# tesseract-robotics/trajopt

Hardware: NVIDIA H100
Metric: converged trajectories/sec (7-DOF x 30 wp, batch 1024) (higher is better)
Workload: dtype f64

## Files before the change

trajopt_b200/csrc/qp_cta_kernel.cuh:

```cuda
#pragma once
#include "device_types.cuh"
#include "joint_terms.cuh"

namespace tb200 {

#ifdef TB200_PROFILE
static __device__ unsigned long long g_prof[32];
#define PROF_T0() const long long prof_t0_ = clock64()
#define PROF_ADD(slot) do { if (q.tid == 0) atomicAdd(&g_prof[slot], (unsigned long long)(clock64() - prof_t0_)); } while (0)
#define PROF_COUNT(slot) do { if (q.tid == 0) atomicAdd(&g_prof[slot], 1ull); } while (0)
#else
#define PROF_T0()
#define PROF_ADD(slot)
#define PROF_COUNT(slot)
#endif
#if defined(TB200_PROFILE) && defined(TB200_PROFILE_CHECK)
#define PROF_CHK_T0() long long pc_ = clock64()
#define PROF_CHK(slot) do { const long long n_ = clock64(); if (q.tid == 0) atomicAdd(&g_prof[slot], (unsigned long long)(n_ - pc_)); pc_ = n_; } while (0)
#else
#define PROF_CHK_T0()
#define PROF_CHK(slot)
#endif

constexpr int kQpThreads = 256;
// ... 709 lines not shown
      if (mine && R.bu_store) w[R.bu_dst] = acc + o;
    }
    __syncthreads();
  }
  if (wbase < R.b0_warps) {
    const double acc = reg_bwd_task<NB>(mB0, (side ? w : v) + R.b0_y, w + R.b0_wl, side, R.b0_hasl, R.b0_hasr);
    const double o = __shfl_xor_sync(0xffffffffu, acc, 1);
    if (R.b0_store) w[R.b0_dst] = acc + o;
  }
  __syncthreads();
}

template <int NB>
__device__ __forceinline__ double p_row(const QpCtx& q, const int i, const double* Dz, const double* vin) {
  constexpr int HB = NB, W = HB + 1;
  const int N = q.N, nbo = q.n_band;
  const double* const Pb = q.Pband;
  const int* const offs = q.band_offs;
  double s = 0.0;
  for (int t0 = 0; t0 < nbo; t0 += 4) {
    double v[4];
#pragma unroll
    for (int u = 0; u < 4; ++u) {
      const int k = (t0 + u < nbo) ? offs[t0 + u] : -1;
      v[u] = (k >= 0 && k <= i) ? (Pb[i * W + k] * Dz[i - k]) * vin[i - k] : 0.0;
    }
    s += v[0]; s += v[1]; s += v[2]; s += v[3];
  }
  for (int t0 = 0; t0 < nbo; t0 += 4) {
    double v[4];
#pragma unroll
    for (int u = 0; u < 4; ++u) {
      const int k = (t0 + u < nbo) ? offs[t0 + u] : -1;
      v[u] = (k >= 1 && i + k < N) ? (Pb[(i + k) * W + k] * Dz[i + k]) * vin[i + k] : 0.0;
    }
    s += v[0]; s += v[1]; s += v[2]; s += v[3];
  }
  return s * (q.c * Dz[i]);
}
template <int NB>
__device__ __forceinline__ void p_matvec(const QpCtx& q, const double* in, double* out) {
  extern __shared__ double sm[];
  const int N = q.N, Np = q.Np;
  const double* const Dz = sm + (q.Dz - q.smbase);
  const double* const vin = sm + (in - q.smbase);
  double* const vout = sm + (out - q.smbase);
  for (int i = q.tid; i < Np; i += kQpThreads) vout[i] = (i < N) ? p_row<NB>(q, i, Dz, vin) : 0.0;
  __syncthreads();
}

__device__ __forceinline__ void info_row_terms(const double* F, const double ax, double (&m)[14]) {
  const double einv = 1.0 / F[R_E];
  m[0] = fmax(m[0], fabs(einv * (ax - F[R_Z])));
  m[1] = fmax(m[1], fabs(einv * F[R_Z]));
  m[2] = fmax(m[2], fabs(einv * ax));
  m[7] = fmax(m[7], fabs(ax - F[R_Z]));
  m[8] = fmax(m[8], fabs(F[R_Z]));
  m[9] = fmax(m[9], fabs(ax));
#pragma unroll
  for (int k = 0; k < 2; ++k) {
    const double u = F[R_U0 + k], bb = F[R_B0 + k], qa = F[R_QA0 + k];
    const double xa = F[R_XA0 + k], za = F[R_ZA0 + k], ya = F[R_YA0 + k];
    const double iea = 1.0 / F[R_EA0 + k], ida = 1.0 / F[R_DA0 + k];
    const double axb = bb * xa;
    m[0] = fmax(m[0], fabs(iea * (axb - za)));
    m[1] = fmax(m[1], fabs(iea * za));
    m[2] = fmax(m[2], fabs(iea * axb));
    m[7] = fmax(m[7], fabs(axb - za));
    m[8] = fmax(m[8], fabs(za));
    m[9] = fmax(m[9], fabs(axb));
    const double aty = u * F[R_Y] + bb * ya;
    m[3] = fmax(m[3], fabs(ida * (qa + aty)));
    m[4] = fmax(m[4], fabs(ida * aty));
    m[5] = fmax(m[5], fabs(ida * qa));
    m[10] = fmax(m[10], fabs(qa + aty));
    m[11] = fmax(m[11], fabs(aty));
    m[12] = fmax(m[12], fabs(qa));
  }
}
__device__ __forceinline__ void info_var_terms(const double dz, const double beta, const double x, const double zb,
                                               const double aty, const double px, const double qv, double (&m)[14]) {
  const double ax = beta * x;
  const double einv = dz / beta, dinv = 1.0 / dz;
  m[0] = fmax(m[0], fabs(einv * (ax - zb)));
  m[1] = fmax(m[1], fabs(einv * zb));
  m[2] = fmax(m[2], fabs(einv * ax));
  m[7] = fmax(m[7], fabs(ax - zb));
  m[8] = fmax(m[8], fabs(zb));
  m[9] = fmax(m[9], fabs(ax));
  const double d = qv + px + aty;
  m[3] = fmax(m[3], fabs(dinv * d));
  m[4] = fmax(m[4], fabs(dinv * aty));
  m[5] = fmax(m[5], fabs(dinv * qv));
  m[6] = fmax(m[6], fabs(dinv * px));
  m[10] = fmax(m[10], fabs(d));
  m[11] = fmax(m[11], fabs(aty));
  m[12] = fmax(m[12], fabs(qv));
  m[13] = fmax(m[13], fabs(px));
}
__device__ __forceinline__ double pinf_row_terms(const double* F, const int naux, double (&a)[3]) {
  double d = F[R_DY];
  d = (naux == AUX_HINGE) ? fmax(d, 0.0) : d;
  a[0] = fmax(a[0], fabs(F[R_E] * d));
  a[1] += F[R_UP] * fmax(d, 0.0) + F[R_LO] * fmin(d, 0.0);
#pragma unroll
  for (int k = 0; k < 2; ++k) {
    const double da = fmin(F[R_DYA0 + k], 0.0);
    a[0] = fmax(a[0], fabs(F[R_EA0 + k] * da));
    a[2] = fmax(a[2], fabs((F[R_U0 + k] * d + F[R_B0 + k] * da) / F[R_DA0 + k]));
  }
  return d;
}
__device__ __forceinline__ void pinf_var_terms(const double ratio, const double ub, const double lb, const double d,
                                               double (&a)[3]) {
  a[0] = fmax(a[0], fabs(ratio * d));
  a[1] += ub * fmax(d, 0.0) + lb * fmin(d, 0.0);
}
__device__ __forceinline__ void dinf_row_terms(const double* F, double (&a)[2]) {
#pragma unroll
  for (int k = 0; k < 2; ++k) {
    a[0] = fmax(a[0], fabs(F[R_DA0 + k] * F[R_DXA0 + k]));
    a[1] += F[R_QA0 + k] * F[R_DXA0 + k];
  }
}
__device__ __forceinline__ unsigned long long guess_mix(unsigned long long v) {
  v += 0x9e3779b97f4a7c15ull;
  v = (v ^ (v >> 30)) * 0xbf58476d1ce4e5b9ull;
  v = (v ^ (v >> 27)) * 0x94d049bb133111ebull;
  return v ^ (v >> 31);
}
__device__ __forceinline__ unsigned long long guess_row_hash(const double* F, const int* I, const int r, const int nrows,
                                                             const int N) {
  unsigned long long h = 0ull;
  const unsigned long long mc = static_cast<unsigned long long>(nrows);
  if (F[R_Z] - F[R_LO] < -F[R_Y]) h += guess_mix(2ull * r);
  else if (F[R_UP] - F[R_Z] < F[R_Y]) h += guess_mix(2ull * r + 1ull);
  for (int k = 0; k < I[RI_AUX]; ++k) {
    const unsigned long long idx = mc + N + I[RI_PAD] + k;
    if (F[R_ZA0 + k] - 0.0 < -F[R_YA0 + k]) h += guess_mix(2ull * idx);
    else if (kOsqpInf * F[R_EA0 + k] - F[R_ZA0 + k] < F[R_YA0 + k]) h += guess_mix(2ull * idx + 1ull);
  }
  return h;
}
__device__ __forceinline__ unsigned long long guess_var_hash(const double zb, const double yb, const double lb,
                                                             const double ub, const int i, const int nrows) {
  const unsigned long long idx = static_cast<unsigned long long>(nrows) + i;
  if (zb - lb < -yb) return guess_mix(2ull * idx);
  if (ub - zb < yb) return guess_mix(2ull * idx + 1ull);
  return 0ull;
}
enum ChkQ { CHK_PA0 = 14, CHK_PA1, CHK_PA2, CHK_DA0, CHK_DA1, kChkHash };
constexpr unsigned kChkSumMask = (1u << CHK_PA1) | (1u << CHK_DA1);

__device__ inline void rows_prepare_weights(const QpCtx& q, const SysW& w) {
  for (int r = q.tid; r < q.nrows; r += kQpThreads) {
    double* F = q.F(r);
    const int naux = q.I(r)[RI_AUX];
    const double Wr = w.polish ? fabs(F[R_PW]) : ((F[R_RHO] != 0.0) ? q.rho_eq : q.rho);
    const double wa0 = w.polish ? fabs(F[R_PWA0]) : w.rho_aux;
    const double wa1 = w.polish ? fabs(F[R_PWA1]) : w.rho_aux;
    const double g0 = (naux >= 1) ? w.sig + wa0 * F[R_B0] * F[R_B0] : 1.0;
    const double g1 = (naux == 2) ? w.sig + wa1 * F[R_B1] * F[R_B1] : 1.0;
    const double den = g0 * g1 + Wr * (F[R_U0] * F[R_U0] * g1 + F[R_U1] * F[R_U1] * g0);
    F[R_WRR] = Wr;
    F[R_G0] = g0;
    F[R_G1] = g1;
    F[R_DEN] = den;
    F[R_IDEN] = 1.0 / den;
    F[R_IWRR] = (Wr != 0.0) ? 1.0 / Wr : 0.0;
    F[R_WR] = Wr * g0 * g1 / den;
  }
  __syncthreads();
}
__device__ __forceinline__ double xbound_weight(const QpCtx& q, const SysW& w, int j) {
  const double adm = (q.ubs[j] - q.lbs[j] < kRhoTol) ? q.rho_eq : q.rho;
  return w.polish ? fabs(q.zb[j]) : adm;
}

__device__ __forceinline__ double pivot_rcp(const double x) {
  double r;
  asm("rcp.approx.ftz.f64 %0, %1;" : "=d"(r) : "d"(x));
  double e = fma(-x, r, 1.0);
  r = fma(r, e, r);
  e = fma(-x, r, 1.0);
  r = fma(r, e, r);
  e = fma(-x, r, 1.0);
  return fma(r, e, r);
}
template <int QN>
__device__ __forceinline__ bool gj_rows(double (&a)[QN], double diag, const bool active, const int mat, const int row,
                                        const int n, const int n_max, double* tmp, const int nmat) {
  constexpr int BS = QN + 2;
  double* const csv = tmp + 2 * nmat * BS + mat * QN;
  bool bad = false;
  double pv_mine = pivot_rcp(diag), my_cs = 1.0, rs = 1.0, inv_rs = 1.0;
#pragma unroll 1
  for (int k = 0; k < n_max; ++k) {
    double* buf = tmp + ((k & 1) * nmat + mat) * BS;
    const bool piv = active && row == k;
    if (piv) {
      bad |= !(diag > 0.0);
#pragma unroll
      for (int j = 0; j < QN; j += 2) *reinterpret_cast<double2*>(buf + j) = make_double2(a[j], a[j + 1]);
      buf[k] = 0.0;
      buf[QN] = pv_mine;
      my_cs = -pv_mine;
      csv[k] = my_cs;
      rs = pv_mine;
      inv_rs = diag;
      diag = pv_mine;
    }
    __syncthreads();
    if (active && k < n && !piv) {
      const double tr = buf[row];
      const bool ahead = row > k;
      const double f = ahead ? tr : -tr * my_cs;
      const double g = f * buf[QN];
      diag = ahead ? diag - g * f : diag + g * f;
      const double gs = g * inv_rs;
#pragma unroll
      for (int j = 0; j < QN; j += 2) {
        const double2 t = *reinterpret_cast<const double2*>(buf + j);
        a[j] -= gs * t.x;
        a[j + 1] -= gs * t.y;
      }
      if (ahead) pv_mine = pivot_rcp(diag);
    }
  }
  if (active) {
#pragma unroll
    for (int j = 0; j < QN; ++j) a[j] = (j == row) ? diag : ((j < n) ? a[j] * (rs * csv[j]) : 0.0);
  }
  return bad;
}

template <int NB>
__device__ inline bool pinv_factor(const QpCtx& q) {
  constexpr int QN = 3 * NB, blk = NB * NB;
  static_assert(QN % 2 == 0, "pivot rows move as double2");
  extern __shared__ double sm[];
  const int tid = q.tid, M = q.M, Np = q.Np;
  const int PR = q.pl.PR, nS = q.pl.nS, Ns = q.pl.Ns, ZS = q.pl.ZS, WS = q.pl.WS, SS = q.pl.SS;
  double* const fbase = sm + (q.SA - q.smbase);
  const double* const SA = fbase;
  const double* const SLM = sm + (q.SLM - q.smbase);
  double* const Z = fbase + q.pl.zo;
  double* const W = fbase + q.pl.wo;
  double* const S = fbase + q.pl.so;
  double* const tmp = q.tmp.ptr();
  const int nparts = (M + 3) / 4;
  bool bad = false;
#ifdef TB200_PROFILE
  long long pf_ = clock64();
#define PROF_PF(slot) do { const long long n_ = clock64(); if (tid == 0) atomicAdd(&g_prof[slot], (unsigned long long)(n_ - pf_)); pf_ = n_; } while (0)
#else
#define PROF_PF(slot)
#endif
  {
    const bool prow = tid < PR;
    const int p = prow ? tid / QN : 0, lr = prow ? tid % QN : 0;
    const int npb = (M - 4 * p) < 3 ? (M - 4 * p) : 3;
    const int kb = lr / NB, r = lr % NB, gb = 4 * p + kb;
    double a[QN];
#pragma unroll
    for (int j = 0; j < QN; ++j) {
      const int cb = j / NB, c = j % NB;
      double v = 0.0;
      if (prow && cb < npb) {
        if (cb == kb) v = SA[gb * blk + r * NB + c];
        else if (cb == kb - 1) v = SLM[gb * blk + r * NB + c];
        else if (cb == kb + 1) v = SLM[(gb + 1) * blk + c * NB + r];
      }
      a[j] = v;
    }
    PROF_PF(0);
    const double dg = prow ? SA[gb * blk + r * NB + r] : 1.0;
    bad |= gj_rows<QN>(a, dg, prow, p, lr, npb * NB, (M < 3 ? M : 3) * NB, tmp, nparts);
    PROF_PF(4);
    if (prow) {
#pragma unroll
      for (int j = 0; j < QN; ++j) q.pi_g[tid * QN + j] = a[j];
      const bool has_l = p > 0, has_r = 4 * p + 3 < M;
#pragma unroll 2
      for (int j = 0; j < NB; ++j) {
        double wl = 0.0, wr = 0.0;
        if (has_l) {
#pragma unroll
          for (int c = 0; c < NB; ++c) wl += a[c] * SLM[(4 * p) * blk + c * NB + j];
        }
        if (has_r) {
#pragma unroll
          for (int c = 0; c < NB; ++c) wr += a[2 * NB + c] * SLM[(4 * p + 3) * blk + j * NB + c];
        }
        W[tid * WS + j] = wl;
        W[tid * WS + NB + j] = wr;
      }
    }
  }
  __syncthreads();
  for (int e = tid; e < nS * nS; e += kQpThreads) {
    const int ra = e / nS, ca = e % nS, sa = ra / NB, i = ra % NB, sb = ca / NB, j = ca % NB;
    double v = 0.0;
    if (sa == sb || sb == sa + 1 || sb == sa - 1) {
      const bool use_l = sb <= sa, use_r = sb >= sa && 4 * sa + 4 < M;
      const double* cl = SLM + (4 * sa + 3) * blk + i * NB;
      const double* wl = W + (sa * QN + 2 * NB) * WS + (sb == sa ? NB : 0) + j;
      const double* cr = SLM + (4 * sa + 4) * blk + i;
      const double* wr = W + ((sa + 1) * QN) * WS + (sb == sa ? 0 : NB) + j;
      double s0 = 0.0, s1 = 0.0, s2 = 0.0, s3 = 0.0;
      if (use_l) {
#pragma unroll
        for (int rr = 0; rr < NB; rr += 2) {
          s0 += cl[rr] * wl[rr * WS];
          s1 += cl[rr + 1] * wl[(rr + 1) * WS];
        }
      }
      if (use_r) {
#pragma unroll
        for (int rr = 0; rr < NB; rr += 2) {
          s2 += cr[rr * NB] * wr[rr * WS];
          s3 += cr[(rr + 1) * NB] * wr[(rr + 1) * WS];
        }
      }
      v = ((sa == sb) ? SA[(4 * sa + 3) * blk + i * NB + j] : 0.0) - ((s0 + s1) + (s2 + s3));
    }
    S[ra * SS + ca] = v;
  }
  __syncthreads();
  PROF_PF(14);
  {
    const bool srow = tid < nS;
    double a[QN];
#pragma unroll
    for (int j = 0; j < QN; ++j) a[j] = (srow && j < nS) ? S[tid * SS + j] : 0.0;
    const double dg = srow ? S[tid * SS + tid] : 1.0;
    bad |= gj_rows<QN>(a, dg, srow, 0, tid, nS, nS, tmp, 1);
    if (srow) {
#pragma unroll
      for (int j = 0; j < QN; ++j)
        if (j < nS) S[tid * SS + j] = a[j];
    }
  }
  __syncthreads();
  PROF_PF(15);
  if (tid < Np) {
    const int col = tid, cb = col / NB, c = col % NB, p = cb / 4;
    if (cb % 4 == 3) {
      for (int sr = 0; sr < nS; ++sr) Z[sr * ZS + col] = S[sr * SS + p * NB + c];
    } else {
      const bool has_l = p > 0, has_r = 4 * p + 3 < M;
      const double* wrow = W + (p * QN + (cb % 4) * NB + c) * WS;
      double wv[2 * NB];
#pragma unroll
      for (int t = 0; t < 2 * NB; ++t) wv[t] = wrow[t];
      const double* sl = S + (has_l ? (p - 1) * NB : 0);
      const double* sr_ = S + (has_r ? p * NB : 0);
#pragma unroll 2
      for (int sr = 0; sr < nS; ++sr) {
        double s0 = 0.0, s1 = 0.0, s2 = 0.0, s3 = 0.0;
#pragma unroll
        for (int t = 0; t < NB; t += 2) {
          s0 += sl[sr * SS + t] * wv[t];
          s1 += sl[sr * SS + t + 1] * wv[t + 1];
          s2 += sr_[sr * SS + t] * wv[NB + t];
          s3 += sr_[sr * SS + t + 1] * wv[NB + t + 1];
        }
        Z[sr * ZS + col] = -((s0 + s1) + (s2 + s3));
      }
    }
  }
  (void)Ns;
  const bool ok = !__syncthreads_or(bad ? 1 : 0);
  PROF_PF(9);
  return ok;
}

template <int NB, bool PINV>
__device__ __noinline__ bool assemble_factor(const QpCtx& q, const SysW& w) {
  PROF_T0();
  rows_prepare_weights(q, w);
  constexpr int nb = NB, blk = NB * NB;
  const int N = q.N, HB = 2 * q.D, PW = HB + 1, CN = q.CN;
  for (int t = q.tid; t < q.M * blk; t += kQpThreads) {
    q.SA[t] = 0.0;
    q.SLM[t] = 0.0;
  }
  __syncthreads();
  for (int i = q.tid; i < q.Np; i += kQpThreads) {
    const int p = i / nb, r = i % nb;
    double* Arow = q.SA + static_cast<size_t>(p) * blk + r * nb;
    double* Lrow = q.SLM + static_cast<size_t>(p) * blk + r * nb;
    if (i >= N) {
      Arow[r] = 1.0;
      continue;
    }
    auto add = [&](int k, double val) {
      if (k <= r) Arow[r - k] += val;
      else Lrow[nb + r - k] += val;
    };
    for (int t = 0; t < q.n_band; ++t) {
      const int k = q.band_offs[t];
      if (k <= i) add(k, q.c * q.Dz[i] * q.Pband[i * PW + k] * q.Dz[i - k]);
    }
    add(0, w.sig + xbound_weight(q, w, i) * q.beta[i] * q.beta[i]);
    for (int e = q.colptr[i]; e < q.colptr[i + 1]; ++e) {
      const int ent = q.colent[e], rw = ent >> 5, k = ent & 31;
      const double* R = q.R(rw);
      const double wr = R[2 * CN + R_WR];
      if (wr == 0.0) continue;
      const int stride = q.I(rw)[RI_STRIDE];
      const double* as = R + CN;
      const double ai = wr * as[k];
      for (int k2 = 0; k2 <= k; ++k2) add((k - k2) * stride, ai * as[k2]);
    }
  }
  __syncthreads();
  for (int t = q.tid; t < q.M * blk; t += kQpThreads) {
    const int p = t / blk, i = (t % blk) / nb, j = t % nb;
    if (j > i) q.SA[static_cast<size_t>(p) * blk + i * nb + j] = q.SA[static_cast<size_t>(p) * blk + j * nb + i];
  }
  __syncthreads();
  PROF_ADD(10);
  bool ok;
  {
    PROF_T0();
    if constexpr (PINV) ok = pinv_factor<NB>(q);
    else ok = bcr_factor<NB>(q);
    PROF_ADD(11);
  }
  return ok;
}

struct QpPlan {
  bool use_reg, use_pinv, fuse, fast_polish;
};
__host__ __device__ inline QpPlan qp_plan(bool regok, int pinv, int rows_smem, int M, int nb, bool fast_passes) {
  QpPlan pl;
  pl.use_reg = regok && solve_roles_fit(M, nb);
  pl.use_pinv = regok && pinv && rows_smem;
  pl.fuse = pl.use_pinv && fast_passes;
  pl.fast_polish = pl.use_pinv && fast_passes && M * nb <= kQpThreads && solve_roles_fit(M, nb);
  return pl;
}
enum QpPath {
  QPP_BLOCK_PINV = 1 << 0,
  QPP_BLOCK_FAST = 1 << 1,
  QPP_BLOCK_GENERIC = 1 << 2,
  QPP_BLOCK_SOA = 1 << 3,
  QPP_FACTOR_GLOBAL = 1 << 4,
  QPP_BAND_GLOBAL = 1 << 5,
  QPP_ROWS_GLOBAL = 1 << 6,
  QPP_FUSED_CHECK = 1 << 7,
  QPP_POLISH_FAST = 1 << 8,
  QPP_POLISH_GENERIC = 1 << 9
};
__host__ __device__ inline int qp_plan_block(const QpPlan& pl, int rows_smem) {
  if (pl.use_pinv) return QPP_BLOCK_PINV;
  if (!rows_smem) return QPP_BLOCK_SOA;
  return pl.use_reg ? QPP_BLOCK_FAST : QPP_BLOCK_GENERIC;
}

struct QpOut {
  int status, iters, polish;
  double rho;
  double pri_res, dua_res, pol_pri, pol_dua, c;
  int pol_factor_ok, rho_updates, rounds;
};

template <int CN, class Base>
__device__ __forceinline__ void scatter_columns(const QpCtx& q, Base base) {
  for (int i = q.tid; i < q.Np; i += kQpThreads) {
    double s = 0.0;
    if (i < q.N) {
      s = base(i);
      for (int e = q.colptr[i]; e < q.colptr[i + 1]; ++e) {
        const int ent = q.colent[e], r = ent >> 5, k = ent & 31;
        const double* R = q.R(r);
        s += R[CN + k] * R[2 * CN + R_COEF];
      }
    }
    q.v1[i] = s;
  }
  __syncthreads();
}
template <int CN>
__device__ __forceinline__ double row_dot(const QpCtx& q, const double* R, const int* I, const double* v) {
  double z = 0.0;
  const int base = I[RI_BASE], stride = I[RI_STRIDE], last = I[RI_CNT] - 1;
#pragma unroll
  for (int k = 0; k < CN; ++k) z += R[CN + k] * v[base + min(k, last) * stride];
  return z;
}
__device__ __forceinline__ void row_backsub(const double* F, double zeta, double& a0, double& a1) {
  const double Wr = F[R_WRR], ra0 = F[R_RA0], ra1 = F[R_RA1], u0 = F[R_U0], u1 = F[R_U1];
  const double iden = F[R_IDEN];
  a0 = (F[R_G1] * (ra0 - Wr * u0 * zeta) + Wr * u1 * (u1 * ra0 - u0 * ra1)) * iden;
  a1 = (F[R_G0] * (ra1 - Wr * u1 * zeta) + Wr * u0 * (u0 * ra1 - u1 * ra0)) * iden;
}
__device__ __forceinline__ double row_reduce_coef(const double* F, double ra0, double ra1, double zcoef) {
  return zcoef - F[R_WRR] * (F[R_U0] * ra0 * F[R_G1] + F[R_U1] * ra1 * F[R_G0]) * F[R_IDEN];
}
template <int CNc>
__device__ __forceinline__ void admm_row_entry(const double* R, double* F, const double& sigma, const double& rho_aux) {
  const double s = F[R_WRR] * F[R_Z] - F[R_Y];
  const double ra0 = sigma * F[R_XA0] - F[R_QA0] + F[R_U0] * s + F[R_B0] * (rho_aux * F[R_ZA0] - F[R_YA0]);
  const double ra1 = sigma * F[R_XA1] - F[R_QA1] + F[R_U1] * s + F[R_B1] * (rho_aux * F[R_ZA1] - F[R_YA1]);
  F[R_RA0] = ra0;
  F[R_RA1] = ra1;
  const double cf = row_reduce_coef(F, ra0, ra1, s);
  F[R_COEF] = cf;
#pragma unroll
  for (int k = 0; k < CNc; ++k) F[R_NF + k] = R[CNc + k] * cf;
}
template <int CNc>
__device__ __forceinline__ void admm_row_update(const double* R, double* F, const int* I, const double* w,
                                                const double& sigma, const double& alpha, const double& oma,
                                                const double& rho_aux, const double& inv_rho_aux) {
  double zeta = 0.0;
  {
    const int base = I[RI_BASE], stride = I[RI_STRIDE], last = I[RI_CNT] - 1;
#pragma unroll
    for (int k = 0; k < CNc; ++k) zeta += R[CNc + k] * w[base + min(k, last) * stride];
  }
  double a0, a1;
  row_backsub(F, zeta, a0, a1);
  const double zt = zeta + F[R_U0] * a0 + F[R_U1] * a1;
  const double Wr = F[R_WRR];
  const double zr = alpha * zt + oma * F[R_Z];
  double zn = zr + F[R_Y] * F[R_IWRR];
  zn = fmin(fmax(zn, F[R_LO]), F[R_UP]);
  const double dy = Wr * (zr - zn);
  const double yn = F[R_Y] + dy;
  F[R_Z] = zn;
  F[R_Y] = yn;
  F[R_DY] = dy;
  const double s = Wr * zn - yn;
  double ra[2];
#pragma unroll
  for (int k = 0; k < 2; ++k) {
    const double at = k ? a1 : a0, bb = F[R_B0 + k];
    const double xo = F[R_XA0 + k];
    const double xn = alpha * at + oma * xo;
    const double zra = alpha * (bb * at) + oma * F[R_ZA0 + k];
    double z2 = zra + F[R_YA0 + k] * inv_rho_aux;
    z2 = fmin(fmax(z2, 0.0), kOsqpInf * F[R_EA0 + k]);
    const double dya = rho_aux * (zra - z2);
    const double yan = F[R_YA0 + k] + dya;
    F[R_XA0 + k] = xn;
    F[R_DXA0 + k] = xn - xo;
    F[R_ZA0 + k] = z2;
    F[R_YA0 + k] = yan;
    F[R_DYA0 + k] = dya;
    ra[k] = sigma * xn - F[R_QA0 + k] + F[R_U0 + k] * s + bb * (rho_aux * z2 - yan);
  }
  F[R_RA0] = ra[0];
  F[R_RA1] = ra[1];
  const double cf = row_reduce_coef(F, ra[0], ra[1], s);
  F[R_COEF] = cf;
#pragma unroll
  for (int k = 0; k < CNc; ++k) F[R_NF + k] = R[CNc + k] * cf;
}

template <int NB, int PAIR>
__device__ __noinline__ void admm_block(const QpCtx& q, const double rho_aux, const int n_iter, const int keep_last) {
  constexpr int CNc = PAIR ? ((NB > 3) ? NB : 3) : ((NB / 2 > 3) ? NB / 2 : 3);
  const int N = q.N, tid = q.tid;
  double* const dxs = q.scratch;
  double* const dyb = q.scratch + q.Np;
  const bool one_var = q.Np <= kQpThreads;
  const int my_e0 = (one_var && tid < N) ? q.colptr[tid] : 0, my_e1 = (one_var && tid < N) ? q.colptr[tid + 1] : 0;
  {
    PROF_T0();
// ... 1016 lines not shown
    } else {
      for (int i = tid; i < N; i += kQpThreads) {
        a[0] = fmax(a[0], fabs(q.Dz[i] * dxs[i]));
        a[1] += q.qs[i] * dxs[i];
      }
      for (int r = tid; r < q.nrows; r += kQpThreads) dinf_row_terms(q.F(r), a);
      block_reduce<2, 0x2u>(q, a);
    }
    const double ndx = a[0], qdx = a[1];
    if (!((ndx > eps) && (qdx < -q.c * eps * ndx))) return false;
    for (int i = tid; i < q.Np; i += kQpThreads) q.v1[i] = (i < N) ? dxs[i] : 0.0;
    __syncthreads();
    p_matvec<NB>(q, q.v1, q.v2);
    double b2[2] = {0.0, 0.0};
    for (int i = tid; i < N; i += kQpThreads) {
      b2[0] = fmax(b2[0], fabs(q.v2[i] / q.Dz[i]));
      const double vv = q.Dz[i] * q.v1[i];
      b2[1] += (vv > eps * ndx || vv < -eps * ndx) ? 1.0 : 0.0;
    }
    for (int r = tid; r < q.nrows; r += kQpThreads) {
      const double* R = q.R(r);
      const double* F = q.F(r);
      const int naux = q.I(r)[RI_AUX];
      const double ax = row_dot<CNc>(q, R, q.I(r), q.v1) + F[R_U0] * F[R_DXA0] + F[R_U1] * F[R_DXA1];
      const double vv = ax / F[R_E];
      b2[1] += (vv > eps * ndx) ? 1.0 : 0.0;
      b2[1] += (naux != AUX_HINGE && vv < -eps * ndx) ? 1.0 : 0.0;
#pragma unroll
      for (int k = 0; k < 2; ++k) {
        const double va = F[R_B0 + k] * F[R_DXA0 + k] / F[R_EA0 + k];
        b2[1] += (k < naux && va < -eps * ndx) ? 1.0 : 0.0;
      }
    }
    block_reduce<2, 0x2u>(q, b2);
    return (ndx > eps) && (qdx < -q.c * eps * ndx) && (b2[0] < q.c * eps * ndx) && (b2[1] == 0.0);
  };
  auto check_termination = [&](bool approximate) -> int {
    double eps_abs = st.eps_abs * eps_scale, eps_rel = st.eps_rel * eps_scale, epi = st.eps_prim_inf, edi = st.eps_dual_inf;
    if (approximate) {
      eps_abs *= 10; eps_rel *= 10; epi *= 10; edi *= 10;
    }
    const double eps_pri = eps_abs + eps_rel * fmax(n_z, n_ax);
    const double eps_dua = eps_abs + eps_rel * q.cinv * fmax(n_q, fmax(n_aty, n_px));
    const bool pri_ok = pri_res < eps_pri, dua_ok = dua_res < eps_dua;
    int res = QPS_UNSOLVED;
    if (pri_res > kOsqpInf || dua_res > kOsqpInf) res = QPS_NONCVX;
    else if (pri_ok && dua_ok) res = approximate ? QPS_SOLVED_INACC : QPS_SOLVED;
    else {
      const bool pinf = pri_ok ? false : primal_infeasible(epi);
      const bool dinf = dua_ok ? false : dual_infeasible(edi);
      if (pinf) res = approximate ? QPS_PINF_INACC : QPS_PINF;
      else if (dinf) res = approximate ? QPS_DINF_INACC : QPS_DINF;
    }
    return res;
  };

  auto early_guess_settled = [&]() -> bool {
    unsigned long long h = 0ull;
    if (fused_chk) {
      extern __shared__ double sm[];
      const unsigned long long* hw = reinterpret_cast<const unsigned long long*>(sm + (q.tmp - q.smbase) + kChkHash * 8);
      for (int w = 0; w < kQpThreads / 32; ++w) h += hw[w];
    } else {
      for (int r = tid; r < q.nrows; r += kQpThreads) h += guess_row_hash(q.F(r), q.I(r), r, q.nrows, N);
      for (int i = tid; i < N; i += kQpThreads) h += guess_var_hash(q.zb[i], q.yb[i], q.lbs[i], q.ubs[i], i, q.nrows);
      __syncwarp();
      for (int off = 16; off > 0; off >>= 1) h += __shfl_xor_sync(0xffffffffu, h, off);
      unsigned long long* red = reinterpret_cast<unsigned long long*>(q.red.ptr());
      if ((tid & 31) == 0) red[tid >> 5] = h;
      __syncthreads();
      h = 0ull;
      for (int w = 0; w < kQpThreads / 32; ++w) h += red[w];
      __syncthreads();
    }
    const bool stable = have_prev_guess && h == prev_guess;
    prev_guess = h;
    have_prev_guess = true;
    pending_guess = h;
    return stable && !(have_failed_guess && h == failed_guess);
  };

  auto run_admm = [&](auto& polish_fn, auto& restore_fn) {
    status = QPS_UNSOLVED;
    bool stop = false;
    while (!stop) {
      if (iter >= st.max_iter) {
        if (!(st.check_termination > 0 && (iter % st.check_termination == 0))) residuals(false);
        status = check_termination(true);
        if (status == QPS_UNSOLVED) status = QPS_MAXITER;
        stop = true;
      } else {
        int n = st.max_iter - iter;
        if (st.check_termination > 0) n = min(n, st.check_termination - iter % st.check_termination);
        if (st.adaptive_rho && st.adaptive_rho_interval > 0) n = min(n, st.adaptive_rho_interval - iter % st.adaptive_rho_interval);
        iter += n;
        const bool can_check = st.check_termination > 0 && (iter % st.check_termination == 0);
        const bool rho_iter = st.adaptive_rho && st.adaptive_rho_interval > 0 && (iter % st.adaptive_rho_interval == 0);
        run_block(n, can_check || iter == st.max_iter);
        if (can_check) {
          PROF_T0();
          residuals(rho_iter);
          PROF_CHK_T0();
          status = check_termination(false);
          PROF_CHK(9);
          PROF_ADD(5);
          bool try_early = false;
          if (status != QPS_UNSOLVED) stop = true;
          else if (st.polishing && st.early_polish_every > 0 && iter >= st.early_polish_from &&
                   (iter % st.early_polish_every == 0)) {
            PROF_T0();
            try_early = early_guess_settled();
            PROF_ADD(22);
          }
          if (try_early) {
            bool verified = false;
            double p_pri = 0.0, p_dua = 0.0;
            PROF_COUNT(17);
            { PROF_T0(); if (use_pinv) stash_z(false); PROF_ADD(16); }
            const bool factored = polish_fn(verified, p_pri, p_dua);
            if (factored && verified) {
              early_verified = true;
              out.pol_factor_ok = 1;
              out.pol_pri = p_pri;
              out.pol_dua = p_dua;
              status = QPS_SOLVED;
              stop = true;
            } else {
              PROF_T0();
              failed_guess = pending_guess;
              have_failed_guess = true;
              restore_fn(false);
              if (use_pinv) {
                stash_z(true);
              } else if (!factorize(sysw)) {
                status = QPS_NONCVX;
                stop = true;
              }
              PROF_ADD(19);
            }
          }
        }
        if (!stop && rho_iter) {
          if (!can_check) residuals(true);
          const double pn = s_pri / (fmax(s_z, s_ax) + 1e-10);
          const double dn = s_dua / (fmax(s_q, fmax(s_aty, s_px)) + 1e-10);
          double rho_new = rho * sqrt(pn / (dn + 1e-10));
          rho_new = fmin(fmax(rho_new, kRhoMin), kRhoMax);
          if (rho_new > rho * st.adaptive_rho_tolerance || rho_new < rho / st.adaptive_rho_tolerance) {
            rho = rho_new;
            q.rho = rho;
            q.rho_eq = kRhoEqOverIneq * rho;
            sysw.rho_aux = rho;
            out.rho_updates++;
            PROF_T0();
            if (!factorize(sysw)) {
              status = QPS_NONCVX;
              stop = true;
            }
            PROF_ADD(20);
          }
        }
      }
    }
  };

  const double wp = 1.0 / st.delta;
  const SysW pw{true, st.delta, 0.0};
  auto polish_refine = [&](bool& verified, double& p_pri, double& p_dua) {
    PROF_T0();
    if constexpr (REGOK) {
      if (fast_polish) {
        using PassFn = PolishRes (*)(const QpCtx&, int);
        PassFn volatile fn = &polish_passes<NB, PAIR>;
        const PolishRes res = fn(q, st.polish_refine_iter);
        p_pri = res.p_pri;
        p_dua = res.p_dua;
        verified = (res.bad == 0.0) && (p_pri <= kVerifyTol) && isfinite(p_pri) && isfinite(p_dua);
        PROF_ADD(12);
        return;
      }
    }
    for (int it = 0; it <= st.polish_refine_iter + 1; ++it) {
      const bool last = (it == st.polish_refine_iter + 1);
      p_matvec<NB>(q, q.x, q.v2);
      double mm[3] = {0.0, 0.0, 0.0};
      for (int r = tid; r < q.nrows; r += kQpThreads) {
        const double* R = q.R(r);
        double* F = q.F(r);
        const int naux = q.I(r)[RI_AUX];
        const double Wr = F[R_WRR];
        const double ax = row_dot<CNc>(q, R, q.I(r), q.x) + F[R_U0] * F[R_PX0] + F[R_U1] * F[R_PX1];
        const double py = F[R_PY] + ((it > 0) ? Wr * (ax - F[R_PB]) : 0.0);
        const double e = py + (last ? 0.0 : Wr * (ax - F[R_PB]));
        const double zc = fmin(fmax(ax, F[R_LO]), F[R_UP]);
        mm[0] = fmax(mm[0], fabs((ax - zc) / F[R_E]));
        mm[2] += (last && Wr != 0.0 && naux == AUX_HINGE && py < -kVerifyTol) ? 1.0 : 0.0;
        double pya[2], ra[2];
#pragma unroll
        for (int k = 0; k < 2; ++k) {
          const double bb = F[R_B0 + k], u = F[R_U0 + k], qa = F[R_QA0 + k];
          const double wa = fabs(F[R_PWA0 + k]);
          const double axb = bb * F[R_PX0 + k];
          pya[k] = F[R_PYA0 + k] + ((it > 0) ? wa * axb : 0.0);
          const double ea = pya[k] + (last ? 0.0 : wa * axb);
          mm[0] = fmax(mm[0], fabs((axb - fmax(axb, 0.0)) / F[R_EA0 + k]));
          mm[2] += (last && wa != 0.0 && pya[k] > kVerifyTol) ? 1.0 : 0.0;
          mm[1] = fmax(mm[1], fabs((qa + u * py + bb * pya[k]) / F[R_DA0 + k]));
          ra[k] = -qa - u * e - bb * ea;
        }
        F[R_PY] = py;
        F[R_PYA0] = pya[0];
        F[R_PYA1] = pya[1];
        F[R_RA0] = ra[0];
        F[R_RA1] = ra[1];
        F[R_COEF] = last ? py : row_reduce_coef(F, ra[0], ra[1], -e);
      }
      __syncthreads();
      if (last) {
        scatter_columns<CNc>(q, [&](int i) { return q.v2[i] + q.qs[i] + q.beta[i] * q.yb[i]; });
      } else {
        scatter_columns<CNc>(q, [&](int i) {
          const double beta = q.beta[i];
          const double w = fabs(q.zb[i]);
          const double bnd = q.zb[i] > 0 ? q.ubs[i] : q.lbs[i];
          return -(q.v2[i] + q.qs[i]) - beta * (q.yb[i] + w * (beta * q.x[i] - bnd));
        });
      }
      for (int i = tid; i < N; i += kQpThreads) {
        const double beta = q.beta[i];
        const double ax = beta * q.x[i];
        const double w = fabs(q.zb[i]);
        const double lb = q.lbs[i], ub = q.ubs[i];
        const double zc = fmin(fmax(ax, lb), ub);
        mm[0] = fmax(mm[0], fabs((ax - zc) * q.Dz[i] / beta));
        const bool ineq = last && w != 0.0 && (ub - lb >= kRhoTol);
        mm[2] += (ineq && q.zb[i] > 0 && q.yb[i] < -kVerifyTol) ? 1.0 : 0.0;
        mm[2] += (ineq && q.zb[i] < 0 && q.yb[i] > kVerifyTol) ? 1.0 : 0.0;
        if (last) mm[1] = fmax(mm[1], fabs(q.v1[i] / q.Dz[i]));
      }
      if (last) {
        block_reduce<3, 0x4u>(q, mm);
        p_pri = mm[0];
        p_dua = mm[1] * q.cinv;
        verified = (mm[2] == 0.0) && (p_pri <= kVerifyTol) && isfinite(p_pri) && isfinite(p_dua);
      } else {
        bcr_solve<NB>(q, q.v1, q.w);
        for (int r = tid; r < q.nrows; r += kQpThreads) {
          const double* R = q.R(r);
          double* F = q.F(r);
          double a0, a1;
          row_backsub(F, row_dot<CNc>(q, R, q.I(r), q.w), a0, a1);
          F[R_PX0] += a0;
          F[R_PX1] += a1;
        }
        for (int i = tid; i < N; i += kQpThreads) {
          const double xn = q.x[i] + q.w[i];
          const double w = fabs(q.zb[i]);
          q.yb[i] += w * (q.beta[i] * xn - (q.zb[i] > 0 ? q.ubs[i] : q.lbs[i]));
          q.x[i] = xn;
        }
        __syncthreads();
      }
    }
    PROF_ADD(12);
  };
  auto polish_once = [&](bool& verified, double& p_pri, double& p_dua) -> bool {
    PROF_COUNT(13);
    PROF_T0();
    verified = false;
    for (int i = tid; i < q.Np; i += kQpThreads) {
      const double z = q.zb[i], y = q.yb[i];
      double w = 0.0;
      if (i < N) {
        if (z - q.lbs[i] < -y) w = -wp;
        else if (q.ubs[i] - z < y) w = wp;
      }
      st_x[i] = q.x[i];
      st_zb[i] = z;
      st_yb[i] = y;
      q.zb[i] = w;
      q.x[i] = 0.0;
      q.yb[i] = 0.0;
    }
    for (int r = tid; r < q.nrows; r += kQpThreads) {
      double* F = q.F(r);
      const int naux = q.I(r)[RI_AUX];
      double w = 0.0, b = 0.0;
      if (F[R_Z] - F[R_LO] < -F[R_Y]) { w = -wp; b = F[R_LO]; }
      else if (F[R_UP] - F[R_Z] < F[R_Y]) { w = wp; b = F[R_UP]; }
      F[R_PW] = w;
      F[R_PB] = b;
      F[R_PY] = 0.0;
#pragma unroll
      for (int k = 0; k < 2; ++k) {
        double wa = 0.0;
        if (k < naux) {
          if (F[R_ZA0 + k] - 0.0 < -F[R_YA0 + k]) wa = -wp;
          else if (kOsqpInf * F[R_EA0 + k] - F[R_ZA0 + k] < F[R_YA0 + k]) wa = wp;
        }
        F[R_PWA0 + k] = wa;
        F[R_PYA0 + k] = 0.0;
        F[R_PX0 + k] = 0.0;
      }
    }
    __syncthreads();
    PROF_ADD(16);
    bool factored;
    { PROF_T0(); factored = factorize(pw); PROF_ADD(23); }
    if (!factored) return false;
    polish_refine(verified, p_pri, p_dua);
    return true;
  };
  auto restore_admm_state = [&](bool keep_polished_x) {
    for (int i = tid; i < q.Np; i += kQpThreads) {
      if (!keep_polished_x) q.x[i] = st_x[i];
      q.zb[i] = st_zb[i];
      q.yb[i] = st_yb[i];
    }
    __syncthreads();
  };

  bool done = !factor_ok;
  while (!done) {
    run_admm(polish_once, restore_admm_state);
    out.pri_res = pri_res;
    out.dua_res = dua_res;
    if (status != QPS_SOLVED || !st.polishing) {
      done = true;
    } else if (early_verified) {
      out.polish = 1;
      out.rounds = round;
      done = true;
    } else {
      bool verified = false;
      double p_pri = 0.0, p_dua = 0.0;
      PROF_COUNT(18);
      { PROF_T0(); if (use_pinv) stash_z(false); PROF_ADD(16); }
      const bool factored = polish_once(verified, p_pri, p_dua);
      out.pol_factor_ok = factored ? 1 : 0;
      out.pol_pri = p_pri;
      out.pol_dua = p_dua;
      out.rounds = round;
      if (factored && verified) {
        out.polish = 1;
        done = true;
      } else if (round >= kVerifyRounds || iter >= st.max_iter) {
        const bool ok = factored && ((p_pri < pri_res && p_dua < dua_res) || (p_pri < pri_res && dua_res < 1e-10) ||
                                     (p_dua < dua_res && pri_res < 1e-10)) && isfinite(p_pri) && isfinite(p_dua);
        out.polish = ok ? 2 : -1;
        done = true;
      } else {
        ++round;
        eps_scale *= 0.1;
        PROF_T0();
        restore_admm_state(false);
        if (use_pinv) {
          stash_z(true);
        } else if (!factorize(sysw)) {
          status = QPS_NONCVX;
          done = true;
        }
        PROF_ADD(19);
      }
    }
  }
  out.iters = iter;
  out.status = status;
  out.rho = rho;
  out.c = q.c;
  if (out.polish != 0) {
    if (out.polish > 0) {
      for (int r = tid; r < q.nrows; r += kQpThreads) {
        double* F = q.F(r);
        for (int k = 0; k < 2; ++k) F[R_XA0 + k] = F[R_PX0 + k];
      }
    }
    restore_admm_state(out.polish > 0);
  }
  return out;
}

template <int DD, int PAIR>
__device__ __noinline__ void qp_step(const DevProblem& p, const int b, const double* x_override ,
                                        const double* trust_override, int* admm_iters_out, int* polish_out) {
  constexpr int NB = 2 * DD;
  constexpr bool FG = DD > 8;
  extern __shared__ double sm[];
  const int tid = threadIdx.x;
  if (!x_override && (p.status[b] != 5 || p.qp_done[b] != 0)) return;
  const int N = p.N, T = p.T, D = p.D;
  QpCtx q;
  q.N = N; q.T = T; q.D = D; q.tid = tid;
  q.nb = NB;
  q.M = qp_block_count(N, NB);
  q.Np = q.M * NB;
  q.CN = (p.row_stride - R_NF) / 3;
  q.RS = p.row_stride;
  const QpSmem S = qp_smem_layout(N, NB, q.RS, q.CN, p.max_rows, FG);
  if (FG || !S.factor_smem) {
    double* fg = p.factor_g + static_cast<size_t>(blockIdx.x) * qp_cta_global_doubles(N, NB);
    const int fb = qp_even(q.M * NB * NB);
    q.SA = fg; q.SLM = fg + fb; q.SU = fg + 2 * fb;
  } else {
    q.SA = sm + S.SA; q.SLM = sm + S.SLM; q.SU = sm + S.SU;
  }
  q.beta = sm + S.beta;
  q.x = sm + S.x; q.zb = sm + S.zb; q.yb = sm + S.yb; q.v1 = sm + S.v1; q.w = sm + S.w;
  q.qs = sm + S.qs; q.lbs = sm + S.lbs; q.ubs = sm + S.ubs; q.tmp = sm + S.tmp; q.red = sm + S.red;
  q.flag = sm + S.red - 8;
  q.colptr = reinterpret_cast<int*>(sm + S.colptr);
  double* const rows_g = p.rows + static_cast<size_t>(b) * p.max_rows * p.row_stride;
  int* const rints_g = p.row_ints + static_cast<size_t>(b) * p.max_rows * RI_NINTS;
  q.rows = rows_g;
  q.soa = p.soa + static_cast<size_t>(blockIdx.x) * p.soa_stride;
  q.smbase = sm;
  q.pinv = S.pinv;
  q.pl = pinv_plan(q.M, NB);
  q.pi_g = p.factor_g + static_cast<size_t>(blockIdx.x) * qp_cta_global_doubles(N, NB);
  q.z_stash = q.pi_g + qp_factor_doubles(N, NB);
  q.rows_smem = 0;
  q.rints = rints_g;
  int* mylist = p.lists + static_cast<size_t>(b) * p.list_stride;
  int* colptr = mylist;
  int* colent = mylist + q.Np + 1;
  int* obj_start = colent + static_cast<size_t>(p.max_rows) * q.CN;
  q.colent = colent;
  q.band_offs = p.band_offs;
  q.n_band = p.n_band;
  if (S.pband_smem) {
    q.Pband = sm + S.Pb;
    for (int t = tid; t < N * (NB + 1); t += kQpThreads) sm[S.Pb + t] = p.Pband[t];
  } else {
    q.Pband = p.Pband;
  }
  double* gvec = p.scratch + static_cast<size_t>(b) * 5 * q.Np;
  q.scratch = gvec;
  q.Dz = sm + S.Dz;
  q.v2 = sm + S.v2;
  double *qs = q.qs, *lbs = q.lbs, *ubs = q.ubs;
  int* meta = p.ws_meta + static_cast<size_t>(b) * 8;
  const int n_obj = p.n_costs + p.n_cnts;
  int nr = 0, n_aux = 0, nnzA = 0;
  bool warm = false;
  int* sh_i = reinterpret_cast<int*>(q.flag + 2);

  {
    const double* xc = (x_override ? x_override : p.x) + static_cast<size_t>(b) * N;
    const double trust = trust_override ? trust_override[b] : p.trust[b];
    const double* mu = p.merit_coeffs + static_cast<size_t>(b) * p.n_cnts;
    const int buf = x_override ? 0 : p.cur_buf[b];
    const size_t slot = static_cast<size_t>(buf) * p.B + b;
    const double* cart_err = p.cart_err + slot * p.n_cart_rows;
    const double* cart_jac = p.cart_jac + slot * static_cast<size_t>(p.n_cart_rows) * p.cart_stride;
    const double* coll_rows = p.coll_rows + slot * static_cast<size_t>(p.n_coll_cand) * p.coll_stride;
    const unsigned long long* coll_mask = p.coll_mask + slot * static_cast<size_t>(p.n_coll_objs) * p.coll_words;

    for (int i = tid; i < N; i += kQpThreads) {
      const double lb = p.lower[i % D], ub = p.upper[i % D];
      const double xi = fmin(fmax(xc[i], lb), ub);
      lbs[i] = fmax(fmax(xi - trust, lb), -kOsqpInf);
// ... 278 lines not shown
```

Before: 1410.

## Assemble block-tridiagonal system in registers with direct shared-memory addressing

Rewrites system assembly so each thread accumulates its row's band entries in a register array, then writes the lower and upper (symmetric) block entries and the zero padding directly. This removes the separate zero-fill pass, the atomic-free read-modify-write accumulation in shared memory, the symmetrisation pass and two barriers. Row and index pointers are also rebased onto the dynamic shared-memory base when the data lives there, so the compiler can emit shared loads instead of generic ones. Profiling slot indices are also renumbered. The cost is larger unrolled register loops with predicated selects, and possible register pressure.

```diff
diff --git a/trajopt_b200/csrc/qp_cta_kernel.cuh b/trajopt_b200/csrc/qp_cta_kernel.cuh
--- a/trajopt_b200/csrc/qp_cta_kernel.cuh
+++ b/trajopt_b200/csrc/qp_cta_kernel.cuh
@@ -885,10 +885,10 @@
 enum ChkQ { CHK_PA0 = 14, CHK_PA1, CHK_PA2, CHK_DA0, CHK_DA1, kChkHash };
 constexpr unsigned kChkSumMask = (1u << CHK_PA1) | (1u << CHK_DA1);
 
-__device__ inline void rows_prepare_weights(const QpCtx& q, const SysW& w) {
+__device__ __forceinline__ void prepare_weights_rows(const QpCtx& q, const SysW& w, double* rows, const int* rints) {
   for (int r = q.tid; r < q.nrows; r += kQpThreads) {
-    double* F = q.F(r);
-    const int naux = q.I(r)[RI_AUX];
+    double* F = rows + static_cast<size_t>(r) * q.RS + 2 * q.CN;
+    const int naux = rints[r * RI_NINTS + RI_AUX];
     const double Wr = w.polish ? fabs(F[R_PW]) : ((F[R_RHO] != 0.0) ? q.rho_eq : q.rho);
     const double wa0 = w.polish ? fabs(F[R_PWA0]) : w.rho_aux;
     const double wa1 = w.polish ? fabs(F[R_PWA1]) : w.rho_aux;
@@ -902,6 +902,15 @@
     F[R_IDEN] = 1.0 / den;
     F[R_IWRR] = (Wr != 0.0) ? 1.0 / Wr : 0.0;
     F[R_WR] = Wr * g0 * g1 / den;
+  }
+}
+__device__ inline void rows_prepare_weights(const QpCtx& q, const SysW& w) {
+  extern __shared__ double sm[];
+  if (q.rows_smem) {
+    prepare_weights_rows(q, w, sm + (q.rows - q.smbase),
+                         reinterpret_cast<const int*>(sm + (reinterpret_cast<const double*>(q.rints) - q.smbase)));
+  } else {
+    prepare_weights_rows(q, w, q.rows, q.rints);
   }
   __syncthreads();
 }
@@ -1006,10 +1015,10 @@
       }
       a[j] = v;
     }
-    PROF_PF(0);
+    PROF_PF(27);
     const double dg = prow ? SA[gb * blk + r * NB + r] : 1.0;
     bad |= gj_rows<QN>(a, dg, prow, p, lr, npb * NB, (M < 3 ? M : 3) * NB, tmp, nparts);
-    PROF_PF(4);
+    PROF_PF(28);
     if (prow) {
 #pragma unroll
       for (int j = 0; j < QN; ++j) q.pi_g[tid * QN + j] = a[j];
@@ -1060,7 +1069,7 @@
     S[ra * SS + ca] = v;
   }
   __syncthreads();
-  PROF_PF(14);
+  PROF_PF(29);
   {
     const bool srow = tid < nS;
     double a[QN];
@@ -1075,7 +1084,7 @@
     }
   }
   __syncthreads();
-  PROF_PF(15);
+  PROF_PF(30);
   if (tid < Np) {
     const int col = tid, cb = col / NB, c = col % NB, p = cb / 4;
     if (cb % 4 == 3) {
@@ -1104,53 +1113,88 @@
   }
   (void)Ns;
   const bool ok = !__syncthreads_or(bad ? 1 : 0);
-  PROF_PF(9);
+  PROF_PF(31);
   return ok;
+}
+
+template <int NB>
+__device__ __forceinline__ void assemble_system(const QpCtx& q, const SysW& w, const double* rows, const int* rints,
+                                                const int* colent, const int* colptr, const double* Pband, double* SA,
+                                                double* SLM) {
+  constexpr int BLK = NB * NB, PW = NB + 1;
+  const int N = q.N, CN = q.CN, RS = q.RS, n_band = q.n_band;
+  const double c = q.c;
+  for (int i = q.tid; i < q.Np; i += kQpThreads) {
+    const int p = i / NB, r = i % NB;
+    double acc[NB + 1];
+#pragma unroll
+    for (int j = 0; j <= NB; ++j) acc[j] = 0.0;
+    if (i >= N) {
+      acc[0] = 1.0;
+    } else {
+      const double dzi = q.Dz[i];
+      for (int t = 0; t < n_band; ++t) {
+        const int k = q.band_offs[t];
+        if (k <= i) {
+          const double v = __dmul_rn(__dmul_rn(__dmul_rn(c, dzi), Pband[i * PW + k]), q.Dz[i - k]);
+#pragma unroll
+          for (int j = 0; j <= NB; ++j)
+            if (j == k) acc[j] = __dadd_rn(acc[j], v);
+        }
+      }
+      const double beta = q.beta[i];
+      acc[0] = __dadd_rn(acc[0], __fma_rn(__dmul_rn(xbound_weight(q, w, i), beta), beta, w.sig));
+      for (int e = colptr[i]; e < colptr[i + 1]; ++e) {
+        const int ent = colent[e], rw = ent >> 5, k = ent & 31;
+        const double* R = rows + static_cast<size_t>(rw) * RS;
+        const double wr = R[2 * CN + R_WR];
+        if (wr == 0.0) continue;
+        const int stride = rints[rw * RI_NINTS + RI_STRIDE];
+        const double* as = R + CN;
+        const double ai = __dmul_rn(wr, as[k]);
+        int nxt = 0, k2 = k;
+#pragma unroll
+        for (int j = 0; j <= NB; ++j) {
+          if (j == nxt && k2 >= 0) {
+            acc[j] = __dadd_rn(acc[j], __dmul_rn(ai, as[k2]));
+            nxt += stride;
+            --k2;
+          }
+        }
+      }
+    }
+    double* const Arow = SA + static_cast<size_t>(p) * BLK + r * NB;
+    double* const Acol = SA + static_cast<size_t>(p) * BLK + r;
+    double* const Lrow = SLM + static_cast<size_t>(p) * BLK + r * NB;
+#pragma unroll
+    for (int j = 0; j <= NB; ++j) {
+      if (j <= r) {
+        Arow[r - j] = acc[j];
+        if (j > 0) Acol[(r - j) * NB] = acc[j];
+      } else {
+        Lrow[NB + r - j] = acc[j];
+      }
+    }
+#pragma unroll
+    for (int c2 = 0; c2 < NB - 1; ++c2)
+      if (c2 < r) Lrow[c2] = 0.0;
+  }
 }
 
 template <int NB, bool PINV>
 __device__ __noinline__ bool assemble_factor(const QpCtx& q, const SysW& w) {
   PROF_T0();
+  PROF_COUNT(26);
   rows_prepare_weights(q, w);
-  constexpr int nb = NB, blk = NB * NB;
-  const int N = q.N, HB = 2 * q.D, PW = HB + 1, CN = q.CN;
-  for (int t = q.tid; t < q.M * blk; t += kQpThreads) {
-    q.SA[t] = 0.0;
-    q.SLM[t] = 0.0;
-  }
-  __syncthreads();
-  for (int i = q.tid; i < q.Np; i += kQpThreads) {
-    const int p = i / nb, r = i % nb;
-    double* Arow = q.SA + static_cast<size_t>(p) * blk + r * nb;
-    double* Lrow = q.SLM + static_cast<size_t>(p) * blk + r * nb;
-    if (i >= N) {
-      Arow[r] = 1.0;
-      continue;
-    }
-    auto add = [&](int k, double val) {
-      if (k <= r) Arow[r - k] += val;
-      else Lrow[nb + r - k] += val;
+  extern __shared__ double sm[];
+  if (q.rows_smem && __isShared(q.SA) && __isShared(q.Pband)) {
+    const auto ints = [&](const int* v) {
+      return reinterpret_cast<const int*>(sm + (reinterpret_cast<const double*>(v) - q.smbase));
     };
-    for (int t = 0; t < q.n_band; ++t) {
-      const int k = q.band_offs[t];
-      if (k <= i) add(k, q.c * q.Dz[i] * q.Pband[i * PW + k] * q.Dz[i - k]);
-    }
-    add(0, w.sig + xbound_weight(q, w, i) * q.beta[i] * q.beta[i]);
-    for (int e = q.colptr[i]; e < q.colptr[i + 1]; ++e) {
-      const int ent = q.colent[e], rw = ent >> 5, k = ent & 31;
-      const double* R = q.R(rw);
-      const double wr = R[2 * CN + R_WR];
-      if (wr == 0.0) continue;
-      const int stride = q.I(rw)[RI_STRIDE];
-      const double* as = R + CN;
-      const double ai = wr * as[k];
-      for (int k2 = 0; k2 <= k; ++k2) add((k - k2) * stride, ai * as[k2]);
-    }
-  }
-  __syncthreads();
-  for (int t = q.tid; t < q.M * blk; t += kQpThreads) {
-    const int p = t / blk, i = (t % blk) / nb, j = t % nb;
-    if (j > i) q.SA[static_cast<size_t>(p) * blk + i * nb + j] = q.SA[static_cast<size_t>(p) * blk + j * nb + i];
+    assemble_system<NB>(q, w, sm + (q.rows - q.smbase), ints(q.rints), ints(q.colent), ints(q.colptr),
+                        sm + (q.Pband - q.smbase), sm + (q.SA - q.smbase), sm + (q.SLM - q.smbase));
+  } else {
+    assemble_system<NB>(q, w, q.rows, q.rints, q.colent, q.colptr, q.Pband, q.SA, q.SLM);
   }
   __syncthreads();
   PROF_ADD(10);
@@ -2473,6 +2517,7 @@
             q.rho_eq = kRhoEqOverIneq * rho;
             sysw.rho_aux = rho;
             out.rho_updates++;
+            PROF_COUNT(24);
             PROF_T0();
             if (!factorize(sysw)) {
               status = QPS_NONCVX;
@@ -2627,6 +2672,7 @@
     __syncthreads();
     PROF_ADD(16);
     bool factored;
+    PROF_COUNT(25);
     { PROF_T0(); factored = factorize(pw); PROF_ADD(23); }
     if (!factored) return false;
     polish_refine(verified, p_pri, p_dua);
```

New measurement: 1427 (median of 6 runs). 1.01x the previous value.
